# marcobellagente93/scaling

Measured on AMD Instinct MI355X. Metric: tokens/sec (whole node) Llama-2-7B-shape bf16, TP×PP×DP on 1/2/4/8 MI355X, higher is better.
Workload: dtype bf16

## Files before the change

csrc/bindings.cpp:

```cpp
#include <torch/extension.h>
#include <ATen/hip/HIPContext.h>
#include <c10/core/DeviceGuard.h>

#include <atomic>
#include <cmath>
#include <cstring>
#include <string>
#include <vector>
#include "kernels/launch.h"

void register_rehearsal(pybind11::module& m);
void register_blaslt(pybind11::module& m);

namespace {

hipStream_t cur_stream() { return at::hip::getCurrentHIPStream().stream(); }

int dt(const at::Tensor& t) {
    switch (t.scalar_type()) {
        case at::kFloat: return DT_F32;
        case at::kBFloat16: return DT_BF16;
        case at::kHalf: return DT_F16;
        default: TORCH_CHECK(false, "scaling_amd: unsupported dtype ", t.scalar_type());
    }
    return -1;
}

void check_cuda(const at::Tensor& t, const char* name) {
    TORCH_CHECK(t.is_cuda(), "scaling_amd: ", name, " must be a GPU tensor");
    TORCH_CHECK(t.is_contiguous(), "scaling_amd: ", name, " must be contiguous");
}

std::vector<at::Tensor> norm_fwd(const at::Tensor& x, const at::Tensor& w, const c10::optional<at::Tensor>& b,
                                 double eps, bool layer, const c10::optional<at::Tensor>& res) {
    check_cuda(x, "x");
    check_cuda(w, "weight");
    const int64_t H = x.size(-1);
    TORCH_CHECK(H % 8 == 0, "norm: hidden size must be a multiple of 8");
    TORCH_CHECK(w.numel() == H && w.scalar_type() == x.scalar_type(), "norm: weight shape/dtype mismatch");
    const int64_t rows = x.numel() / H;
    const at::DeviceGuard g(x.device());
    auto y = at::empty_like(x);
    auto opts = x.options().dtype(at::kFloat);
    auto rstd = at::empty({rows}, opts);
    auto mean = layer ? at::empty({rows}, opts) : at::empty({0}, opts);
    const void* bp = nullptr;
    if (layer) {
        TORCH_CHECK(b.has_value(), "layernorm needs a bias");
        check_cuda(*b, "bias");
        bp = b->data_ptr();
    }
    at::Tensor sum = at::empty({0}, x.options());
    const void* rp = nullptr;
    if (res.has_value()) {
        check_cuda(*res, "residual");
        TORCH_CHECK(res->sizes() == x.sizes() && res->scalar_type() == x.scalar_type(), "norm: residual mismatch");
        sum = at::empty_like(x);
        rp = res->data_ptr();
    }
    sa_launch::norm_fwd(dt(x), layer, x.data_ptr(), w.data_ptr(), bp, y.data_ptr(),
                        layer ? mean.data_ptr<float>() : nullptr, rstd.data_ptr<float>(), rows, (int)H, (float)eps,
// ... 311 lines not shown
    const int64_t M = x.size(0), K = W.size(1), N = epi == 2 ? W.size(0) / 2 : W.size(0);
    const at::DeviceGuard g(x.device());
    at::Tensor s = x;
    const void* ap = nullptr;
    if (add.has_value() && add->defined()) {
        TORCH_CHECK(add->sizes() == x.sizes() && add->is_contiguous() && add->scalar_type() == x.scalar_type() &&
                        (uintptr_t)add->data_ptr() % 16 == 0, "gemv_norm: add must be a contiguous, aligned [M, K]");
        s = at::empty_like(x);
        ap = add->data_ptr();
    }
    auto y = at::empty({M, N}, x.options());
    sa_launch::gemv(dt(x), (int)M, x.data_ptr(), x.stride(0), W.data_ptr(), W.stride(0), nullptr, y.data_ptr(), N, (int)N,
                    (int)K, cur_stream(), (int)epi, nullptr, 0, gamma.data_ptr(), ap, ap ? s.data_ptr() : nullptr,
                    (float)eps);
    return {s, y};
}
c10::optional<at::Tensor> gemv_norm_rope(const at::Tensor& x, const at::Tensor& gamma, double eps, const at::Tensor& W,
                                         const at::Tensor& cosb, const at::Tensor& sinb, const at::Tensor& pos,
                                         int64_t nq, int64_t nkv, int64_t rd, at::Tensor kc, at::Tensor vc,
                                         at::Tensor err) {
    TORCH_CHECK(err_word(err), "gemv_norm_rope: err must be an int32 GPU tensor");
    if (!gemv_norm_ok(x, W, gamma) || x.size(0) != 1) return c10::nullopt;
    if (!(kc.is_cuda() && kc.dim() == 3 && kc.is_contiguous() && vc.is_contiguous() && vc.sizes() == kc.sizes() &&
          kc.size(1) == nkv && kc.scalar_type() == x.scalar_type() && vc.scalar_type() == x.scalar_type()))
        return c10::nullopt;
    const int64_t hd = kc.size(2);
    if (hd % 2 || rd % 2 || rd > hd || W.size(0) != (nq + 2 * nkv) * hd) return c10::nullopt;
    if (!(pos.is_cuda() && pos.scalar_type() == at::kLong && pos.numel() == 1 && cosb.scalar_type() == at::kFloat &&
          sinb.scalar_type() == at::kFloat && cosb.is_contiguous() && sinb.is_contiguous() && cosb.size(-1) == rd / 2 &&
          sinb.sizes() == cosb.sizes()))
        return c10::nullopt;
    const at::DeviceGuard g(x.device());
    auto q = at::empty({1, nq, hd}, x.options());
    GemvRope r{cosb.data_ptr<float>(), sinb.data_ptr<float>(), pos.data_ptr<int64_t>(), q.data_ptr(), kc.data_ptr(),
               vc.data_ptr(), (int)nq, (int)nkv, (int)hd, (int)rd, std::min<int64_t>(kc.size(0), cosb.size(0)),
               err.data_ptr<int>()};
    sa_launch::gemv(dt(x), 1, x.data_ptr(), x.stride(0), W.data_ptr(), W.stride(0), nullptr, nullptr, 0,
                    (int)W.size(0), (int)W.size(1), cur_stream(), 3, nullptr, 0, gamma.data_ptr(), nullptr, nullptr,
                    (float)eps, &r);
    return q;
}

bool gemm_tn_ok(const at::Tensor& A, const at::Tensor& B, const at::Tensor& C) {
    if (!(A.is_cuda() && B.is_cuda() && C.is_cuda() && A.dim() == 2 && B.dim() == 2 && C.dim() == 2)) return false;
    if (A.scalar_type() != at::kBFloat16 || B.scalar_type() != at::kBFloat16 || C.scalar_type() != at::kBFloat16)
        return false;
    if (A.stride(1) != 1 || B.stride(1) != 1 || C.stride(1) != 1 || A.size(0) != B.size(0) || C.size(0) != A.size(1) ||
        C.size(1) != B.size(1))
        return false;
    for (const at::Tensor* t : {&A, &B}) if ((uintptr_t)t->data_ptr() % 16 != 0) return false;
    if ((uintptr_t)C.data_ptr() % 8 != 0) return false;
    return sa_launch::gemm_tn_supported(A.size(1), B.size(1), A.size(0), A.stride(0), B.stride(0), C.stride(0));
}
void gemm_tn(const at::Tensor& A, const at::Tensor& B, const at::Tensor& C, bool accumulate) {
    TORCH_CHECK(gemm_tn_ok(A, B, C), "gemm_tn: unsupported operands (bf16 2-D, M/N multiples of 16, K of 128)");
    const at::DeviceGuard g(A.device());
    static int slots = -1;
    if (slots < 0) {
        hipDeviceProp_t prop;
        slots = hipGetDeviceProperties(&prop, A.device().index()) == hipSuccess ? prop.multiProcessorCount : 0;
    }
    int full_blocks = -1, split = 1;
    const int64_t ws_floats = sa_launch::gemm_tn_plan(A.size(1), B.size(1), A.size(0), slots, full_blocks, split);
    at::Tensor ws;
    if (ws_floats > 0) ws = at::empty({ws_floats}, A.options().dtype(at::kFloat));
    sa_launch::gemm_tn(A.data_ptr(), A.stride(0), B.data_ptr(), B.stride(0), C.data_ptr(), C.stride(0), A.size(1),
                       B.size(1), A.size(0), accumulate, cur_stream(), full_blocks, split,
                       ws_floats > 0 ? ws.data_ptr<float>() : nullptr);
}

void check_qkv(const at::Tensor& t, const char* n) {
    TORCH_CHECK(t.is_cuda() && t.dim() == 3 && t.stride(2) == 1, "flash_attn: ", n, " must be [T, heads, D] with unit last stride");
    TORCH_CHECK(t.scalar_type() == at::kBFloat16 || t.scalar_type() == at::kHalf, "flash_attn: ", n, " must be bfloat16 or float16");
    TORCH_CHECK(t.stride(1) % 8 == 0 && t.stride(0) % 8 == 0, "flash_attn: ", n, " strides must be multiples of 8");
}
uint32_t drop_threshold(double p) {
    const double t = p * 4294967296.0;
    return t >= 4294967295.0 ? 0xffffffffu : (uint32_t)t;
}
std::vector<at::Tensor> fa_fwd(const at::Tensor& q, const at::Tensor& k, const at::Tensor& v, const at::Tensor& cu_q,
                               const at::Tensor& cu_k, int64_t max_q, double scale, bool causal, int64_t window,
                               double p_drop, int64_t seed, int64_t local_heads, int64_t max_k) {
    check_qkv(q, "q"); check_qkv(k, "k"); check_qkv(v, "v");
    TORCH_CHECK(k.scalar_type() == q.scalar_type() && v.scalar_type() == q.scalar_type(), "flash_attn: q/k/v dtypes differ");
    TORCH_CHECK(p_drop >= 0.0 && p_drop < 1.0, "flash_attn: dropout probability must be in [0, 1)");
    const int64_t D = q.size(2);
    TORCH_CHECK(D == 32 || D == 64 || D == 128, "flash_attn: head dim must be 32, 64 or 128");
    TORCH_CHECK(k.size(2) == D && v.size(2) == D && k.size(1) == v.size(1) && q.size(1) % k.size(1) == 0, "flash_attn: shapes");
    TORCH_CHECK(cu_q.scalar_type() == at::kInt && cu_k.scalar_type() == at::kInt && cu_q.numel() == cu_k.numel(), "flash_attn: cu_seqlens int32");
    const at::DeviceGuard g(q.device());
    const int64_t T = q.size(0), H = q.size(1);
    auto o = at::empty({T, H, D}, q.options());
    auto lse = at::empty({H, T}, q.options().dtype(at::kFloat));
    FwdArgs a{};
    a.q = (const uint16_t*)q.data_ptr(); a.k = (const uint16_t*)k.data_ptr(); a.v = (const uint16_t*)v.data_ptr();
    a.o = (uint16_t*)o.data_ptr(); a.lse = lse.data_ptr<float>();
    a.q_tok = q.stride(0); a.q_head = q.stride(1); a.k_tok = k.stride(0); a.k_head = k.stride(1);
    a.v_tok = v.stride(0); a.v_head = v.stride(1); a.o_tok = o.stride(0); a.o_head = o.stride(1); a.lse_stride = T;
    a.cu_q = cu_q.data_ptr<int>(); a.cu_k = cu_k.data_ptr<int>();
    a.nseg = (int)cu_q.numel() - 1; a.Hq = (int)H; a.Hkv = (int)k.size(1); a.causal = causal ? 1 : 0; a.window = (int)window;
    a.local_heads = local_heads < 0 ? (int)H : (int)local_heads;
    a.scale_log2 = (float)(scale * 1.4426950408889634);
    a.p_drop = (float)p_drop; a.rp_drop = (float)(1.0 / (1.0 - p_drop)); a.seed = (uint32_t)seed; a.drop_thr = drop_threshold(p_drop);
    const int64_t grp = H / k.size(1);
    if (T > 0 && a.nseg > 0 && p_drop == 0.0 && max_q * grp <= 32) {
        DecArgs d{};
        d.q = a.q; d.k = a.k; d.v = a.v;
        d.q_tok = a.q_tok; d.q_head = a.q_head; d.k_tok = a.k_tok; d.k_head = a.k_head; d.v_tok = a.v_tok; d.v_head = a.v_head;
        d.cu_q = a.cu_q; d.cu_k = a.cu_k; d.nseg = a.nseg; d.Hq = a.Hq; d.Hkv = a.Hkv; d.causal = a.causal;
        d.window = a.window; d.local_heads = a.local_heads; d.scale_log2 = a.scale_log2; d.Tq = T;
        sa_launch::fa_decode_plan(max_k > 0 ? max_k : k.size(0), a.Hkv, a.nseg, d.split_keys, d.nsplit);
        auto part_o = at::empty({(int64_t)d.nsplit, T, H, D}, q.options().dtype(at::kFloat));
        auto part_ml = at::empty({(int64_t)d.nsplit, T, H, 2}, q.options().dtype(at::kFloat));
        d.part_o = part_o.data_ptr<float>(); d.part_ml = part_ml.data_ptr<float>();
        d.o = a.o; d.o_tok = a.o_tok; d.o_head = a.o_head; d.lse = a.lse; d.lse_stride = a.lse_stride;
        sa_launch::fa_decode(d, (int)D, q.scalar_type() == at::kHalf, cur_stream());
        return {o, lse};
    }
    if (T > 0 && a.nseg > 0) sa_launch::fa_fwd(a, (int)D, (int)max_q, q.scalar_type() == at::kHalf, cur_stream());
    return {o, lse};
}
// ... 192 lines not shown
    TORCH_CHECK(logits.stride(1) == 1 || V == 1, "sample: logits need a unit last stride");
    TORCH_CHECK(B <= 1 || logits.stride(0) >= 0, "sample: negative row stride");
    TORCH_CHECK(step.is_cuda() && step.scalar_type() == at::kLong && step.numel() == 1 &&
                step.device() == logits.device(), "sample: step must be one int64 on the logits' device");
    TORCH_CHECK(temperature > 0.0 && std::isfinite(temperature), "sample: temperature must be positive");
    TORCH_CHECK(!std::isnan(top_p), "sample: top_p is NaN");
    const int code = dt(logits);
    const at::DeviceGuard g(logits.device());
    auto tokens = at::empty({B}, logits.options().dtype(at::kLong));
    at::Tensor info;
    if (want_info) info = at::empty({B, 2}, logits.options().dtype(at::kInt));
    if (B > 0)
        sa_launch::sample(code, logits.data_ptr(), B > 1 ? logits.stride(0) : 0, B, (int)V, tokens.data_ptr<int64_t>(),
                          want_info ? info.data_ptr<int>() : nullptr, step.data_ptr<int64_t>(), (uint32_t)seed,
                          (int)std::max<int64_t>(0, std::min<int64_t>(top_k, V)), (float)std::max(top_p, 0.0),
                          (float)temperature, cur_stream());
    if (want_info) return {tokens, info};
    return {tokens};
}
}

PYBIND11_MODULE(TORCH_EXTENSION_NAME, m) {
    m.def("sample_logits", &sample_logits, "one draw per row of logits [B, V] after top-k / top-p / temperature "
          "(graph-safe: the step is read on the device)", py::arg("logits"), py::arg("step"), py::arg("seed"),
          py::arg("temperature"), py::arg("top_k"), py::arg("top_p"), py::arg("want_info") = false);
    m.def("sample_max_resident_vocab", []() { return sa_launch::sample_max_resident(); },
          "the largest vocabulary whose row the sampling kernel stages in LDS");
    m.doc() = "scaling_amd CDNA4 (gfx950) HIP kernels";
    register_rehearsal(m);
    register_blaslt(m);
    m.def("norm_fwd", &norm_fwd, "RMSNorm/LayerNorm forward (optional fused residual add)", py::arg("x"), py::arg("w"), py::arg("b"), py::arg("eps"), py::arg("layer"), py::arg("res") = py::none());
    m.def("norm_bwd", &norm_bwd, "RMSNorm/LayerNorm backward (optional fused residual-gradient add)", py::arg("dy"), py::arg("x"), py::arg("w"), py::arg("mean"), py::arg("rstd"), py::arg("layer"), py::arg("dadd") = py::none());
    m.def("swiglu_fwd", &swiglu_fwd, "SwiGLU forward");
    m.def("swiglu_bwd", &swiglu_bwd, "SwiGLU backward");
    m.def("ar_alloc", &ar_alloc, "one-shot all-reduce: allocate + IPC-export a registered buffer");
    m.def("ar_open", &ar_open, "one-shot all-reduce: map a peer's registered buffer");
    m.def("ar_close", &ar_close, "unmap a peer buffer");
    m.def("ar_free", &ar_free, "free an own registered buffer");
    m.def("ar_allreduce", &ar_allreduce, "one-shot all-reduce of x over the registered buffers (in place)",
          py::arg("x"), py::arg("bases"), py::arg("rank"), py::arg("slot_off"), py::arg("flag_off"), py::arg("epoch"),
          py::arg("signal"), py::arg("err"), py::arg("max_spins") = int64_t(1) << 26);
    m.def("transpose_ok", &transpose_ok, "whether transpose2d supports this tensor");
    m.def("transpose2d", &transpose2d, "x^T (contiguous) for 2-byte 2-D matrices");
    m.def("gemv_ok", &gemv_ok, "whether gemv supports these operands");
    m.def("gemv", &gemv, "y = x W^T (+ b) for at most 4 rows of x (decode-time linear layers)", py::arg("x"), py::arg("W"), py::arg("bias") = py::none());
    m.def("gemv_residual", &gemv_residual, "y = x W^T + res for at most 4 rows (decode MLP-out + residual)");
    m.def("gemv_swiglu", &gemv_swiglu, "y = silu(x Wg^T) * (x Wu^T) for W = [Wg; Wu], at most 4 rows (decode)");
    m.def("gemv_norm_ok", &gemv_norm_ok, "whether gemv_norm supports these operands");
    m.def("gemv_norm_rope", &gemv_norm_rope, "graph decode: rms_norm + q/k/v GEMV + interleaved RoPE + K/V cache append "
          "in one launch; returns q or None");
    m.def("gemv_norm", &gemv_norm, "(s, gemv(rms_norm(s), W)) with s = x (+ add); epi 0 plain, 2 SwiGLU (decode)",
          py::arg("x"), py::arg("add"), py::arg("gamma"), py::arg("eps"), py::arg("W"), py::arg("epi") = 0);
    m.def("gemm_tn_ok", &gemm_tn_ok, "whether gemm_tn supports these operands");
    m.def("gemm_tn", &gemm_tn, "C (+)= A^T B for k-major bf16 operands (weight-gradient GEMM)");
    m.def("rope", &rope, "rotary embedding (fwd / inverse), optional strided / in-place output", py::arg("x"), py::arg("cos"), py::arg("sin"), py::arg("pos"), py::arg("rot_dim"), py::arg("seq_len"), py::arg("interleaved"), py::arg("inverse"), py::arg("out") = py::none());
    m.def("rope_kv_append", &rope_kv_append, "graph decode: RoPE q, RoPE k into the K cache row, v into the V cache row");
    m.def("xent_stats", &xent_stats, "cross-entropy row statistics");
    m.def("xent_bwd", &xent_bwd, "cross-entropy backward");
    m.def("embed_fwd", &embed_fwd, "vocab-parallel embedding forward");
    m.def("embed_bwd", &embed_bwd, "deterministic embedding backward", py::call_guard<py::gil_scoped_release>());
    m.def("adamw_", &adamw_, "fused AdamW on flat fp32 buffers");
    m.def("sumsq_", &sumsq_, "sum of squares + non-finite count");
    m.def("cast_scale_", &cast_scale_, "y = cast(x * scale)");
    m.def("masked_softmax_fwd", &masked_softmax_fwd, "softmax(masked_fill(x * scale, mask, fill)) over the last dim", py::arg("x"), py::arg("mask"), py::arg("scale"), py::arg("fill"), py::arg("round_scaled"));
    m.def("masked_softmax_bwd", &masked_softmax_bwd, "masked softmax backward", py::arg("dy"), py::arg("y"), py::arg("mask"), py::arg("scale"));
    m.def("act_fwd", &act_fwd, "activation forward (0 gelu, 1 silu, 2 gelu-tanh)");
    m.def("act_bwd", &act_bwd, "activation backward");
    m.def("spin_us", &spin_us, "debug: busy-wait kernel of ~us microseconds on the current stream");
    m.def("gate_flags_alloc", &gate_flags_alloc, "stream gates: n flag words (coherent pinned host memory)");
    m.def("gate_flag_write", &gate_flag_write, "stream gates: host store of a flag word (after a full fence)");
    m.def("gate_flag_read", &gate_flag_read, "stream gates: host load of a flag word");
    m.def("gate_stream_wait", &gate_stream_wait, "stream gates: the current stream waits until flag[idx] >= value");
    m.def("xgmi_emulate", &xgmi_emulate, "per-rank proxy: emulated collective (HBM traffic on nwg CUs, held to us)",
          py::arg("src"), py::arg("scratch"), py::arg("bytes"), py::arg("us"), py::arg("nwg") = 16);
    m.def("dropout_add", &dropout_add, "residual + dropout(x) with a hashed keep mask", py::arg("x"), py::arg("res"), py::arg("p"), py::arg("seed"));
    m.def("fa_fwd", &fa_fwd, "flash attention forward (bf16/fp16, optional attention dropout)", py::arg("q"), py::arg("k"), py::arg("v"), py::arg("cu_q"), py::arg("cu_k"), py::arg("max_q"), py::arg("scale"), py::arg("causal"), py::arg("window"), py::arg("p_drop") = 0.0, py::arg("seed") = 0, py::arg("local_heads") = -1, py::arg("max_k") = -1);
    m.def("fa_bwd", &fa_bwd, "flash attention backward (optional strided dq/dk/dv outputs)", py::arg("dout"), py::arg("q"), py::arg("k"), py::arg("v"), py::arg("o"), py::arg("lse"), py::arg("cu_q"), py::arg("cu_k"), py::arg("max_q"), py::arg("max_k"), py::arg("scale"), py::arg("causal"), py::arg("window"), py::arg("dq_out") = py::none(), py::arg("dk_out") = py::none(), py::arg("dv_out") = py::none(), py::arg("p_drop") = 0.0, py::arg("seed") = 0, py::arg("local_heads") = -1, py::arg("rope_cos") = py::none(), py::arg("rope_sin") = py::none(), py::arg("rope_pos") = py::none(), py::arg("rope_dim") = 0, py::arg("rope_seq") = 1, py::arg("rope_interleaved") = false);
}
```

csrc/kernels/gemm.hip:

```cpp
#include <algorithm>

#include "common.h"
#include "flash_attn.h"
#include "launch.h"

using namespace sa;

namespace sa_gemm {

using fa::bf16x8;
using fa::lds_s16x4;
using fa::lds_void;

__host__ __device__ __forceinline__ int group_m(int tm, int tn) {
#ifdef SA_WGRAD_GROUPM
    (void)tm;
    (void)tn;
    return SA_WGRAD_GROUPM;
#else
    return tm >= 2 * tn ? 4 : 8;
#endif
}
constexpr int BK = 32;
constexpr int kImg = BK * 256 * 2;
constexpr int kSlot = 2 * kImg;
constexpr int kSlots = 4;
constexpr int NW = 4;
constexpr int NP = kImg / 1024 / NW;

template <int N>
__device__ __forceinline__ void wait_vm() {
    asm volatile("s_waitcnt vmcnt(%0)" ::"n"(N) : "memory");
}
__device__ __forceinline__ void hard_barrier() {
    __builtin_amdgcn_sched_barrier(0);
    asm volatile("s_barrier" ::: "memory");
    __builtin_amdgcn_sched_barrier(0);
}
__device__ __forceinline__ void mfma16_acc(f32x4& c, const bf16x8& a, const bf16x8& b) {
    asm volatile("v_mfma_f32_16x16x32_bf16 %0, %1, %2, %0" : "+a"(c) : "v"(a), "v"(b));
}
__device__ __forceinline__ int sw16(int r) { return ((r & 3) << 2) ^ (((r >> 2) & 1) << 1); }
__device__ __forceinline__ int koff16(int r, int c) { return r * 512 + 16 * ((c >> 3) ^ sw16(r)) + ((c & 7) << 1); }

#ifndef SA_WGRAD_ROUND
#define SA_WGRAD_ROUND 1
#endif
__device__ __forceinline__ int round_remap(int b, int nwg) {
    if constexpr (SA_WGRAD_ROUND) {
        constexpr int R = 256;
        const int full = nwg / R * R;
        if (b >= full) return full + xcd_remap(b - full, nwg - full);
        return b / R * R + xcd_remap(b % R, R);
    }
    return xcd_remap(b, nwg);
}

template <bool BETA>
__global__ __launch_bounds__(256, 1) void gemm_tn_ring_kernel(const u16* __restrict__ A, int lda, uint32_t a_bytes,
                                                              const u16* __restrict__ B, int ldb, uint32_t b_bytes,
                                                              u16* __restrict__ C, int ldc, int M, int N, int K,
                                                              int full_blocks, int tail_split, float* __restrict__ ws) {
    extern __shared__ __attribute__((aligned(16))) char smem[];
    const int lane = threadIdx.x & 63;
    const int wave = __builtin_amdgcn_readfirstlane(threadIdx.x >> 6);
    const int wm = wave >> 1, wn = wave & 1;

    const int tm = (M + 255) / 256, tn = (N + 255) / 256;
    int v, k_lo = 0, nk = K / 64, unit = -1;
    if ((int)blockIdx.x < full_blocks) {
        v = round_remap(blockIdx.x, full_blocks);
    } else {
        unit = (int)blockIdx.x - full_blocks;
        v = full_blocks + unit / tail_split;
        nk /= tail_split;
        k_lo = (unit % tail_split) * nk;
    }
    const int ns = 2 * nk, s_lo = 2 * k_lo;
    const int gM = group_m(tm, tn);
    const int group = gM * tn;
    const int first_m = (v / group) * gM;
    const int gm = min(tm - first_m, gM);
    const int within = v % group;
    const int m0 = (first_m + within % gm) * 256, n0 = (within / gm) * 256;

    int voff_a, voff_b, step_a, step_b;
    {
        const int row = 2 * wave + (lane >> 5);
        const int slot = (lane & 31) ^ sw16(row);
        voff_a = (row * lda + slot * 8) * 2;
        voff_b = (row * ldb + slot * 8) * 2;
        step_a = __builtin_amdgcn_readfirstlane(4 * NW * lda);
        step_b = __builtin_amdgcn_readfirstlane(4 * NW * ldb);
    }
    auto soff_a = [&](int u) { return __builtin_amdgcn_readfirstlane(((s_lo + min(u, ns - 1)) * BK * lda + m0) * 2); };
    auto soff_b = [&](int u) { return __builtin_amdgcn_readfirstlane(((s_lo + min(u, ns - 1)) * BK * ldb + n0) * 2); };
    typedef int i32x4 __attribute__((ext_vector_type(4)));
    const i32x4 rsa = {(int)__builtin_amdgcn_readfirstlane((uint32_t)reinterpret_cast<uint64_t>(A)),
                       (int)(__builtin_amdgcn_readfirstlane((uint32_t)(reinterpret_cast<uint64_t>(A) >> 32)) & 0xffff),
                       (int)__builtin_amdgcn_readfirstlane(a_bytes), fa::kBufFlags};
    const i32x4 rsb = {(int)__builtin_amdgcn_readfirstlane((uint32_t)reinterpret_cast<uint64_t>(B)),
                       (int)(__builtin_amdgcn_readfirstlane((uint32_t)(reinterpret_cast<uint64_t>(B) >> 32)) & 0xffff),
                       (int)__builtin_amdgcn_readfirstlane(b_bytes), fa::kBufFlags};
    const uint32_t lds0 = __builtin_amdgcn_readfirstlane((uint32_t)reinterpret_cast<uintptr_t>((lds_void*)smem));
#define SA_RING_PIECE(P, SLOT, SA, SB)                                                                           \
    {                                                                                                            \
        const int i_ = (P) >> 1;                                                                                 \
        const uint32_t l_ = lds0 + (SLOT) * kSlot + (((P) & 1) ? kImg : 0) + (wave + NW * i_) * 1024;            \
        if ((P) & 1)                                                                                             \
            asm volatile("s_mov_b32 m0, %0\n\ts_nop 0\n\tbuffer_load_dwordx4 %1, %2, %3 offen lds" ::"s"(l_),    \
                         "v"(voff_b), "s"(rsb), "s"((SB) + i_ * step_b)                                       \
                         : "m0");                                                                                \
        else                                                                                                     \
            asm volatile("s_mov_b32 m0, %0\n\ts_nop 0\n\tbuffer_load_dwordx4 %1, %2, %3 offen lds" ::"s"(l_),    \
                         "v"(voff_a), "s"(rsa), "s"((SA) + i_ * step_a)                                       \
                         : "m0");                                                                                \
    }
#define SA_RING_MFMA_PIECE(C_, A_, B_, P, SLOT, SA, SB)                                                          \
    {                                                                                                            \
        const int i_ = (P) >> 1;                                                                                 \
        const uint32_t l_ = lds0 + (SLOT) * kSlot + (((P) & 1) ? kImg : 0) + (wave + NW * i_) * 1024;            \
        if ((P) & 1)                                                                                             \
            asm volatile("s_mov_b32 m0, %3\n\tv_mfma_f32_16x16x32_bf16 %0, %1, %2, %0\n\t"                     \
                         "buffer_load_dwordx4 %4, %5, %6 offen lds"                                              \
                         : "+a"(C_) : "v"(A_), "v"(B_), "s"(l_), "v"(voff_b), "s"(rsb), "s"((SB) + i_ * step_b)  \
                         : "m0");                                                                                \
        else                                                                                                     \
            asm volatile("s_mov_b32 m0, %3\n\tv_mfma_f32_16x16x32_bf16 %0, %1, %2, %0\n\t"                     \
                         "buffer_load_dwordx4 %4, %5, %6 offen lds"                                              \
                         : "+a"(C_) : "v"(A_), "v"(B_), "s"(l_), "v"(voff_a), "s"(rsa), "s"((SA) + i_ * step_a)  \
                         : "m0");                                                                                \
    }

    f32x4 acc[8][8];
#pragma unroll
    for (int i = 0; i < 8; ++i)
#pragma unroll
        for (int j = 0; j < 8; ++j) acc[i][j] = f32x4{0.f, 0.f, 0.f, 0.f};

    int oa[2][8], ob[2][8];
    {
        const int g = lane >> 4, i16 = lane & 15;
        const int row = 4 * g + (i16 >> 2), cl = 4 * (i16 & 3);
#pragma unroll
        for (int h = 0; h < 2; ++h)
#pragma unroll
            for (int i = 0; i < 8; ++i) {
                oa[h][i] = h * 2 * kSlot + koff16(row, 128 * wm + 16 * i + cl);
                ob[h][i] = h * 2 * kSlot + kImg + koff16(row, 128 * wn + 16 * i + cl);
            }
    }
    auto frag = [&](int off, int slot) -> bf16x8 {
        const char* p = smem + off + (slot & 1) * kSlot;
        const s16x4 x = __builtin_amdgcn_ds_read_tr16_b64_v4i16((lds_s16x4*)p);
        const s16x4 y = __builtin_amdgcn_ds_read_tr16_b64_v4i16((lds_s16x4*)(p + 16 * 512));
        return __builtin_bit_cast(bf16x8, __builtin_shufflevector(x, y, 0, 1, 2, 3, 4, 5, 6, 7));
    };
    bf16x8 fa0[8], fb0[8], fa1[8], fb1[8];
#define SA_RING_READ(SLOT, FA, FB, F)                                         \
    {                                                                         \
        if ((F) < 8) FB[(F)] = frag(ob[(SLOT) >> 1][(F)], (SLOT));            \
        else FA[(F) - 8] = frag(oa[(SLOT) >> 1][(F) - 8], (SLOT));            \
    }
#define SA_RING_STEP(SLOT, T, FA, FB, NA, NB)                                                                   \
    {                                                                                                           \
        const int sa_ = soff_a((T) + 4), sb_ = soff_b((T) + 4);                                                 \
        _Pragma("unroll") for (int i = 0; i < 8; ++i)                                                           \
            _Pragma("unroll") for (int j = 0; j < 8; ++j) {                                                     \
                const int m_ = i * 8 + j;                                                                       \
                if ((m_ & 7) == 3) SA_RING_MFMA_PIECE(acc[i][j], FB[j], FA[i], m_ >> 3, SLOT, sa_, sb_)         \
                else mfma16_acc(acc[i][j], FB[j], FA[i]);                                                       \
                if ((m_ & 3) == 1) SA_RING_READ(((SLOT) + 1) & 3, NA, NB, m_ >> 2)                              \
            }                                                                                                   \
        asm volatile("s_waitcnt lgkmcnt(0)" ::: "memory");                                                      \
        wait_vm<4 * NP>();                                                                                      \
        hard_barrier();                                                                                         \
    }

    asm volatile("s_nop 4" ::: "memory");
#pragma unroll
    for (int u = 0; u < 4; ++u) {
        const int sa_ = soff_a(u), sb_ = soff_b(u);
#pragma unroll
        for (int p = 0; p < 8; ++p) SA_RING_PIECE(p, u, sa_, sb_)
    }
    wait_vm<4 * NP>();
    hard_barrier();
#pragma unroll
    for (int f = 0; f < 16; ++f) SA_RING_READ(0, fa0, fb0, f)
    asm volatile("s_waitcnt lgkmcnt(0)" ::: "memory");
    hard_barrier();
    for (int t = 0; t + 3 < ns; t += 4) {
        SA_RING_STEP(0, t, fa0, fb0, fa1, fb1)
        SA_RING_STEP(1, t + 1, fa1, fb1, fa0, fb0)
        SA_RING_STEP(2, t + 2, fa0, fb0, fa1, fb1)
        SA_RING_STEP(3, t + 3, fa1, fb1, fa0, fb0)
    }
#undef SA_RING_STEP
#undef SA_RING_READ
#undef SA_RING_PIECE
#undef SA_RING_MFMA_PIECE
    wait_vm<0>();
    asm volatile("s_nop 7\n\ts_nop 7\n\ts_nop 7" ::: "memory");
#pragma unroll
    for (int i = 0; i < 8; ++i)
#pragma unroll
        for (int j = 0; j < 8; ++j) asm volatile("" : "+a"(acc[i][j]));

    const int r = lane & 15, q4 = 4 * (lane >> 4);
    if (unit >= 0) {
        float* wp = ws + (int64_t)unit * 65536;
#pragma unroll
        for (int i = 0; i < 8; ++i) {
            float* rp = wp + (128 * wm + 16 * i + r) * 256 + 128 * wn + q4;
#pragma unroll
            for (int j = 0; j < 8; ++j) *reinterpret_cast<f32x4*>(rp + 16 * j) = acc[i][j];
        }
        return;
    }
    const bool edge = m0 + 256 > M || n0 + 256 > N;
#pragma unroll
    for (int i = 0; i < 8; ++i) {
        if (edge && m0 + 128 * wm + 16 * i >= M) continue;
        u16* crow_p = C + (int64_t)(m0 + 128 * wm + 16 * i + r) * ldc + n0 + 128 * wn + q4;
        u16x4 old[8];
        if (BETA) {
#pragma unroll
            for (int j = 0; j < 8; ++j)
                if (!edge || n0 + 128 * wn + 16 * j < N) old[j] = *reinterpret_cast<const u16x4*>(crow_p + 16 * j);
        }
#pragma unroll
        for (int j = 0; j < 8; ++j) {
            if (edge && n0 + 128 * wn + 16 * j >= N) continue;
            u16x4 o;
#pragma unroll
            for (int e = 0; e < 4; ++e) {
                float x = acc[i][j][e];
                if (BETA) x += bf2f(old[j][e]);
                o[e] = f2bf(x);
            }
            *reinterpret_cast<u16x4*>(crow_p + 16 * j) = o;
        }
    }
}
template __global__ void gemm_tn_ring_kernel<true>(const u16* __restrict__, int, uint32_t, const u16* __restrict__, int,
                                                   uint32_t, u16* __restrict__, int, int, int, int, int, int,
                                                   float* __restrict__);
template __global__ void gemm_tn_ring_kernel<false>(const u16* __restrict__, int, uint32_t, const u16* __restrict__, int,
                                                    uint32_t, u16* __restrict__, int, int, int, int, int, int,
                                                    float* __restrict__);

__global__ __launch_bounds__(256) void gemm_tn_combine_kernel(const float* __restrict__ ws, u16* __restrict__ C, int ldc,
                                                              int M, int N, int full_blocks, int split, int beta) {
    const int tm = (M + 255) / 256, tn = (N + 255) / 256;
    const int v = full_blocks + (int)blockIdx.x;
    const int gM = group_m(tm, tn);
    const int group = gM * tn;
    const int first_m = (v / group) * gM;
    const int gm = min(tm - first_m, gM);
    const int within = v % group;
    const int m0 = (first_m + within % gm) * 256, n0 = (within / gm) * 256;
    const int row = 4 * (int)blockIdx.y + (threadIdx.x >> 6), col = (threadIdx.x & 63) * 4;
    if (m0 + row >= M || n0 + col >= N) return;
    f32x4 acc = {0.f, 0.f, 0.f, 0.f};
    const float* wp = ws + (int64_t)blockIdx.x * split * 65536 + row * 256 + col;
    for (int p = 0; p < split; ++p) {
        const f32x4 x = *reinterpret_cast<const f32x4*>(wp + (int64_t)p * 65536);
        acc += x;
    }
    u16* cp = C + (int64_t)(m0 + row) * ldc + n0 + col;
    u16x4 o;
    const u16x4 old = beta ? *reinterpret_cast<const u16x4*>(cp) : u16x4{0, 0, 0, 0};
#pragma unroll
    for (int e = 0; e < 4; ++e) o[e] = f2bf(acc[e] + (beta ? bf2f(old[e]) : 0.f));
    *reinterpret_cast<u16x4*>(cp) = o;
}

}
using namespace sa_gemm;

namespace sa_launch {
bool gemm_tn_supported(int64_t M, int64_t N, int64_t K, int64_t lda, int64_t ldb, int64_t ldc) {
    return M % 16 == 0 && N % 16 == 0 && K % 128 == 0 && M > 0 && N > 0 && K > 0 && lda % 8 == 0 &&
           ldb % 8 == 0 && ldc % 4 == 0 && K * lda * 2 < (int64_t(1) << 31) && K * ldb * 2 < (int64_t(1) << 31) &&
           ldc < (1 << 30);
}
int64_t gemm_tn_plan(int64_t M, int64_t N, int64_t K, int slots, int& full_blocks, int& split) {
    const int nwg = (int)(((M + 255) / 256) * ((N + 255) / 256));
    full_blocks = nwg;
    split = 1;
    if (slots <= 0) return 0;
    const int r = nwg % slots, nk = (int)(K / 64);
    if (r == 0 || nk % 2 != 0) return 0;
    int s = 1;
    double best = 1.0;
    for (int c = 2; c <= 4; ++c) {
        if (nk % c != 0 || nk / c < 4 || (nk / c) % 2 != 0) continue;
        const double cost = (double)((r * c + slots - 1) / slots) / c;
        if (cost < best - 1e-9) { best = cost; s = c; }
    }
    if (s <= 1 || best > 0.8) return 0;
    split = s;
    full_blocks = nwg - r;
    return (int64_t)r * s * 65536;
}
void gemm_tn(const void* A, int64_t lda, const void* B, int64_t ldb, void* C, int64_t ldc, int64_t M, int64_t N,
             int64_t K, bool beta, hipStream_t st, int full_blocks, int split, float* ws) {
    const int nwg = (int)(((M + 255) / 256) * ((N + 255) / 256));
    if (full_blocks < 0 || split <= 1) { full_blocks = nwg; split = 1; }
    const int grid = full_blocks + (nwg - full_blocks) * split;
    const uint32_t ab = (uint32_t)(K * lda * 2), bb = (uint32_t)(K * ldb * 2);
    if (beta)
        hipLaunchKernelGGL((gemm_tn_ring_kernel<true>), dim3(grid), dim3(256), kSlots * kSlot, st, (const u16*)A,
                           (int)lda, ab, (const u16*)B, (int)ldb, bb, (u16*)C, (int)ldc, (int)M, (int)N, (int)K,
                           full_blocks, split, ws);
    else
        hipLaunchKernelGGL((gemm_tn_ring_kernel<false>), dim3(grid), dim3(256), kSlots * kSlot, st, (const u16*)A,
                           (int)lda, ab, (const u16*)B, (int)ldb, bb, (u16*)C, (int)ldc, (int)M, (int)N, (int)K,
                           full_blocks, split, ws);
    if (split > 1)
        hipLaunchKernelGGL(gemm_tn_combine_kernel, dim3(nwg - full_blocks, 64), dim3(256), 0, st, (const float*)ws,
                           (u16*)C, (int)ldc, (int)M, (int)N, full_blocks, split, beta ? 1 : 0);
}
}
```

csrc/kernels/launch.h:

```cpp
#pragma once
#include <hip/hip_runtime.h>
#include <stdint.h>

enum SaDType { DT_F32 = 0, DT_BF16 = 1, DT_F16 = 2 };

namespace sa_launch {
void norm_fwd(int dtype, bool layer, const void* x, const void* w, const void* b, void* y, float* mean, float* rstd,
              int64_t rows, int H, float eps, hipStream_t st, const void* res = nullptr, void* sum_out = nullptr);
int norm_bwd_waves(int64_t rows, int H);
int64_t norm_bwd_scratch(int64_t rows, int H, bool layer);
void norm_bwd(int dtype, bool layer, const void* dy, const void* x, const void* w, const float* mean,
              const float* rstd, void* dx, void* dw, void* db, float* part, int64_t rows, int H, hipStream_t st,
              const void* dadd = nullptr);
}

namespace sa_launch {
void swiglu_fwd(int dtype, const void* a, const void* b, int64_t lda, void* out, int64_t rows, int F, hipStream_t st);
void swiglu_bwd(int dtype, const void* dy, const void* a, const void* b, int64_t lda, void* da, void* db, int64_t ldd,
                int64_t rows, int F, hipStream_t st);
void rope(int dtype, bool interleaved, const void* x, int64_t x_tok, int64_t x_head, void* out, int64_t o_tok,
          int64_t o_head, const float* cosb, const float* sinb, const int64_t* pos, int64_t T_, int nh, int hd, int rd,
          int seq_len, float sign, hipStream_t st);
bool rope_kv_append(int dtype, bool interleaved, const void* x, void* q_out, void* kc, void* vc, const int64_t* pos,
                    const float* cosb, const float* sinb, int nq, int nkv, int hd, int rd, int64_t lim, int* err,
                    hipStream_t st);
}

namespace sa_launch {
void xent_stats(int dtype, const void* logits, const int64_t* tgt, int64_t rows, int V, int64_t v0, float* m, float* s,
                float* t, int64_t* amax, hipStream_t st);
void xent_bwd(int dtype, const void* logits, const int64_t* tgt, const float* lse, const float* gscale, void* dlogits,
              int64_t rows, int V, int64_t v0, hipStream_t st);
void embed_fwd(int dtype, const int64_t* ids, const void* W, void* out, int64_t ntok, int H, int64_t v0, int64_t Vp,
               hipStream_t st);
void embed_bwd(int dtype, const void* dy, const int64_t* order, const int64_t* sid, int64_t ntok, void* dW, int H,
               int64_t v0, int64_t Vp, hipStream_t st);
void adamw(int gdtype, int pdtype, float* p, const void* g, float* m, float* v, void* pout, int64_t n, float lr,
           float b1, float b2, float eps, float wd, float bc1, float bc2_sqrt, float gscale, hipStream_t st);
int sumsq_blocks(int64_t n);
void sumsq(int dtype, const void* x, int64_t n, float scale, float* part_sq, float* part_bad, float* out_sq,
           float* out_bad, int accumulate, hipStream_t st);
void cast_scale(int sdt, int ddt, const void* x, void* y, int64_t n, float scale, hipStream_t st);
bool transpose_supported(int64_t R, int64_t C, int64_t ld_in);
void transpose_u16(const void* in, int64_t ld_in, void* out, int64_t R, int64_t C, hipStream_t st);
}

namespace sa_launch {
bool gemm_tn_supported(int64_t M, int64_t N, int64_t K, int64_t lda, int64_t ldb, int64_t ldc);
int64_t gemm_tn_plan(int64_t M, int64_t N, int64_t K, int slots, int& full_blocks, int& split);
void gemm_tn(const void* A, int64_t lda, const void* B, int64_t ldb, void* C, int64_t ldc, int64_t M, int64_t N,
             int64_t K, bool beta, hipStream_t st, int full_blocks = -1, int split = 1, float* ws = nullptr);
}

struct FwdArgs {
    const uint16_t* q; const uint16_t* k; const uint16_t* v; uint16_t* o; float* lse;
    int64_t q_tok, q_head, k_tok, k_head, v_tok, v_head, o_tok, o_head, lse_stride;
    const int* cu_q; const int* cu_k;
    int nseg, Hq, Hkv, causal, window;
    int local_heads;
    float scale_log2;
    float p_drop, rp_drop;
    uint32_t seed, drop_thr;
};
namespace sa_launch {
void fa_fwd(const FwdArgs& a, int D, int max_q, bool f16, hipStream_t st);
}

struct DecArgs {
    const uint16_t* q; const uint16_t* k; const uint16_t* v;
    int64_t q_tok, q_head, k_tok, k_head, v_tok, v_head;
    const int* cu_q; const int* cu_k;
    int nseg, Hq, Hkv, causal, window, local_heads;
    float scale_log2;
    int split_keys, nsplit;
    int64_t Tq;
    float* part_o;
    float* part_ml;
    uint16_t* o; int64_t o_tok, o_head;
    float* lse; int64_t lse_stride;
};
namespace sa_launch {
void fa_decode_plan(int64_t max_k, int Hkv, int nseg, int& split_keys, int& nsplit);
void fa_decode(const DecArgs& a, int D, bool f16, hipStream_t st);
}

struct BwdArgs {
    const uint16_t* q; const uint16_t* k; const uint16_t* v; const uint16_t* dO;
    const float* lse; float* delta; float* lse2;
    uint16_t* dq; uint16_t* dk; uint16_t* dv;
    int64_t q_tok, q_head, k_tok, k_head, v_tok, v_head, do_tok, do_head;
    int64_t dq_tok, dq_head, dk_tok, dk_head, dv_tok, dv_head, lse_stride;
    const int* cu_q; const int* cu_k;
    int nseg, Hq, Hkv, causal, window;
    int local_heads;
    float scale, scale_log2;
    float p_drop, rp_drop;
    uint32_t seed, drop_thr;
    int hsplit, Tk;
    float* dk_part;
    float* dv_part;
    const float* rcos; const float* rsin; const int64_t* rpos;
    int rrd, rseq, ril;
};
namespace sa_launch {
// ... 43 lines not shown
```

Baseline: 33110.

## Replace split-K tail plan with stream-K style chunk balancing for gemm_tn

The weight-gradient GEMM's last partial wave used to be split into 2-4 equal K pieces per tile. It is now handled by distributing every K chunk of the tail tiles evenly over all workgroup slots, so a workgroup may cover parts of several tiles. Each segment writes an fp32 partial to its own workspace slot, and the combine kernel sums a tile's range of slots. A cost model decides whether the tail split pays off, and the slot count can be overridden. The intent is to remove tail-wave underutilisation, at the cost of extra workspace traffic and a combine launch.

Result: no change. 33170 (median of 6 runs) (+0.2%).

```diff
diff --git a/csrc/bindings.cpp b/csrc/bindings.cpp
--- a/csrc/bindings.cpp
+++ b/csrc/bindings.cpp
@@ -7,6 +7,7 @@
 #include <cstring>
 #include <string>
 #include <vector>
+#include "kernels/gemm_tn_plan.h"
 #include "kernels/launch.h"
 
 void register_rehearsal(pybind11::module& m);
@@ -424,21 +425,22 @@
     if ((uintptr_t)C.data_ptr() % 8 != 0) return false;
     return sa_launch::gemm_tn_supported(A.size(1), B.size(1), A.size(0), A.stride(0), B.stride(0), C.stride(0));
 }
-void gemm_tn(const at::Tensor& A, const at::Tensor& B, const at::Tensor& C, bool accumulate) {
+void gemm_tn(const at::Tensor& A, const at::Tensor& B, const at::Tensor& C, bool accumulate, int64_t slots) {
     TORCH_CHECK(gemm_tn_ok(A, B, C), "gemm_tn: unsupported operands (bf16 2-D, M/N multiples of 16, K of 128)");
+    TORCH_CHECK(slots >= -1 && slots <= 4096, "gemm_tn: slots must be -1 (the device's CU count) or 0..4096");
     const at::DeviceGuard g(A.device());
-    static int slots = -1;
-    if (slots < 0) {
+    static int cus = -1;
+    if (cus < 0) {
         hipDeviceProp_t prop;
-        slots = hipGetDeviceProperties(&prop, A.device().index()) == hipSuccess ? prop.multiProcessorCount : 0;
-    }
-    int full_blocks = -1, split = 1;
-    const int64_t ws_floats = sa_launch::gemm_tn_plan(A.size(1), B.size(1), A.size(0), slots, full_blocks, split);
+        cus = hipGetDeviceProperties(&prop, A.device().index()) == hipSuccess ? prop.multiProcessorCount : 0;
+    }
+    const int s = slots < 0 ? cus : (int)slots;
+    const int64_t ws_floats =
+        sa_gemm_plan::workspace_floats(sa_gemm_plan::make_plan(A.size(1), B.size(1), A.size(0), s));
     at::Tensor ws;
     if (ws_floats > 0) ws = at::empty({ws_floats}, A.options().dtype(at::kFloat));
     sa_launch::gemm_tn(A.data_ptr(), A.stride(0), B.data_ptr(), B.stride(0), C.data_ptr(), C.stride(0), A.size(1),
-                       B.size(1), A.size(0), accumulate, cur_stream(), full_blocks, split,
-                       ws_floats > 0 ? ws.data_ptr<float>() : nullptr);
+                       B.size(1), A.size(0), accumulate, cur_stream(), s, ws_floats > 0 ? ws.data_ptr<float>() : nullptr);
 }
 
 void check_qkv(const at::Tensor& t, const char* n) {
@@ -737,7 +739,9 @@
     m.def("gemv_norm", &gemv_norm, "(s, gemv(rms_norm(s), W)) with s = x (+ add); epi 0 plain, 2 SwiGLU (decode)",
           py::arg("x"), py::arg("add"), py::arg("gamma"), py::arg("eps"), py::arg("W"), py::arg("epi") = 0);
     m.def("gemm_tn_ok", &gemm_tn_ok, "whether gemm_tn supports these operands");
-    m.def("gemm_tn", &gemm_tn, "C (+)= A^T B for k-major bf16 operands (weight-gradient GEMM)");
+    m.def("gemm_tn", &gemm_tn, "C (+)= A^T B for k-major bf16 operands (weight-gradient GEMM); slots: workgroup slots "
+          "the tail of the last round is planned for (-1: the device's CU count)", py::arg("A"), py::arg("B"),
+          py::arg("C"), py::arg("accumulate"), py::arg("slots") = -1);
     m.def("rope", &rope, "rotary embedding (fwd / inverse), optional strided / in-place output", py::arg("x"), py::arg("cos"), py::arg("sin"), py::arg("pos"), py::arg("rot_dim"), py::arg("seq_len"), py::arg("interleaved"), py::arg("inverse"), py::arg("out") = py::none());
     m.def("rope_kv_append", &rope_kv_append, "graph decode: RoPE q, RoPE k into the K cache row, v into the V cache row");
     m.def("xent_stats", &xent_stats, "cross-entropy row statistics");
diff --git a/csrc/kernels/gemm.hip b/csrc/kernels/gemm.hip
--- a/csrc/kernels/gemm.hip
+++ b/csrc/kernels/gemm.hip
@@ -2,6 +2,7 @@
 
 #include "common.h"
 #include "flash_attn.h"
+#include "gemm_tn_plan.h"
 #include "launch.h"
 
 using namespace sa;
@@ -60,29 +61,35 @@
 __global__ __launch_bounds__(256, 1) void gemm_tn_ring_kernel(const u16* __restrict__ A, int lda, uint32_t a_bytes,
                                                               const u16* __restrict__ B, int ldb, uint32_t b_bytes,
                                                               u16* __restrict__ C, int ldc, int M, int N, int K,
-                                                              int full_blocks, int tail_split, float* __restrict__ ws) {
+                                                              sa_gemm_plan::Plan plan, float* __restrict__ ws) {
     extern __shared__ __attribute__((aligned(16))) char smem[];
     const int lane = threadIdx.x & 63;
     const int wave = __builtin_amdgcn_readfirstlane(threadIdx.x >> 6);
     const int wm = wave >> 1, wn = wave & 1;
 
     const int tm = (M + 255) / 256, tn = (N + 255) / 256;
-    int v, k_lo = 0, nk = K / 64, unit = -1;
-    if ((int)blockIdx.x < full_blocks) {
-        v = round_remap(blockIdx.x, full_blocks);
-    } else {
-        unit = (int)blockIdx.x - full_blocks;
-        v = full_blocks + unit / tail_split;
-        nk /= tail_split;
-        k_lo = (unit % tail_split) * nk;
-    }
-    const int ns = 2 * nk, s_lo = 2 * k_lo;
+    const int unit = (int)blockIdx.x - plan.full_blocks;
+    const int nseg = unit >= 0 ? sa_gemm_plan::segment_count(plan, unit) : 1;
     const int gM = group_m(tm, tn);
     const int group = gM * tn;
-    const int first_m = (v / group) * gM;
-    const int gm = min(tm - first_m, gM);
-    const int within = v % group;
-    const int m0 = (first_m + within % gm) * 256, n0 = (within / gm) * 256;
+    int m0 = 0, n0 = 0, s_lo = 0, ns = K / BK, pslot = 0;
+    auto set_segment = [&](int sg) {
+        int v;
+        if (unit < 0) {
+            v = round_remap(blockIdx.x, plan.full_blocks);
+        } else {
+            const sa_gemm_plan::Segment s = sa_gemm_plan::segment(plan, unit, sg);
+            v = plan.full_blocks + sa_gemm_plan::tail_tile_order(plan, s.tile);
+            s_lo = __builtin_amdgcn_readfirstlane(4 * s.first_chunk);
+            ns = __builtin_amdgcn_readfirstlane(4 * s.chunks);
+            pslot = __builtin_amdgcn_readfirstlane(s.slot);
+        }
+        const int first_m = (v / group) * gM;
+        const int gm = min(tm - first_m, gM);
+        const int within = v % group;
+        m0 = (first_m + within % gm) * 256;
+        n0 = (within / gm) * 256;
+    };
 
     int voff_a, voff_b, step_a, step_b;
     {
@@ -133,10 +140,6 @@
     }
 
     f32x4 acc[8][8];
-#pragma unroll
-    for (int i = 0; i < 8; ++i)
-#pragma unroll
-        for (int j = 0; j < 8; ++j) acc[i][j] = f32x4{0.f, 0.f, 0.f, 0.f};
 
     int oa[2][8], ob[2][8];
     {
@@ -177,47 +180,55 @@
         hard_barrier();                                                                                         \
     }
 
-    asm volatile("s_nop 4" ::: "memory");
-#pragma unroll
-    for (int u = 0; u < 4; ++u) {
-        const int sa_ = soff_a(u), sb_ = soff_b(u);
-#pragma unroll
-        for (int p = 0; p < 8; ++p) SA_RING_PIECE(p, u, sa_, sb_)
-    }
-    wait_vm<4 * NP>();
-    hard_barrier();
-#pragma unroll
-    for (int f = 0; f < 16; ++f) SA_RING_READ(0, fa0, fb0, f)
-    asm volatile("s_waitcnt lgkmcnt(0)" ::: "memory");
-    hard_barrier();
-    for (int t = 0; t + 3 < ns; t += 4) {
-        SA_RING_STEP(0, t, fa0, fb0, fa1, fb1)
-        SA_RING_STEP(1, t + 1, fa1, fb1, fa0, fb0)
-        SA_RING_STEP(2, t + 2, fa0, fb0, fa1, fb1)
-        SA_RING_STEP(3, t + 3, fa1, fb1, fa0, fb0)
+    const int r = lane & 15, q4 = 4 * (lane >> 4);
+    for (int sg = 0;; ++sg) {
+        set_segment(sg);
+#pragma unroll
+        for (int i = 0; i < 8; ++i)
+#pragma unroll
+            for (int j = 0; j < 8; ++j) acc[i][j] = f32x4{0.f, 0.f, 0.f, 0.f};
+        asm volatile("s_nop 4" ::: "memory");
+#pragma unroll
+        for (int u = 0; u < 4; ++u) {
+            const int sa_ = soff_a(u), sb_ = soff_b(u);
+#pragma unroll
+            for (int p = 0; p < 8; ++p) SA_RING_PIECE(p, u, sa_, sb_)
+        }
+        wait_vm<4 * NP>();
+        hard_barrier();
+#pragma unroll
+        for (int f = 0; f < 16; ++f) SA_RING_READ(0, fa0, fb0, f)
+        asm volatile("s_waitcnt lgkmcnt(0)" ::: "memory");
+        hard_barrier();
+        for (int t = 0; t + 3 < ns; t += 4) {
+            SA_RING_STEP(0, t, fa0, fb0, fa1, fb1)
+            SA_RING_STEP(1, t + 1, fa1, fb1, fa0, fb0)
+            SA_RING_STEP(2, t + 2, fa0, fb0, fa1, fb1)
+            SA_RING_STEP(3, t + 3, fa1, fb1, fa0, fb0)
+        }
+        wait_vm<0>();
+        asm volatile("s_nop 7\n\ts_nop 7\n\ts_nop 7" ::: "memory");
+#pragma unroll
+        for (int i = 0; i < 8; ++i)
+#pragma unroll
+            for (int j = 0; j < 8; ++j) asm volatile("" : "+a"(acc[i][j]));
+        if (unit < 0) break;
+        float* wp = ws + (int64_t)pslot * sa_gemm_plan::kTileFloats;
+#pragma unroll
+        for (int i = 0; i < 8; ++i) {
+            float* rp = wp + (128 * wm + 16 * i + r) * 256 + 128 * wn + q4;
+#pragma unroll
+            for (int j = 0; j < 8; ++j) *reinterpret_cast<f32x4*>(rp + 16 * j) = acc[i][j];
+        }
+        if (sg + 1 >= nseg) return;
+        asm volatile("s_waitcnt lgkmcnt(0)" ::: "memory");
+        hard_barrier();
     }
 #undef SA_RING_STEP
 #undef SA_RING_READ
 #undef SA_RING_PIECE
 #undef SA_RING_MFMA_PIECE
-    wait_vm<0>();
-    asm volatile("s_nop 7\n\ts_nop 7\n\ts_nop 7" ::: "memory");
-#pragma unroll
-    for (int i = 0; i < 8; ++i)
-#pragma unroll
-        for (int j = 0; j < 8; ++j) asm volatile("" : "+a"(acc[i][j]));
-
-    const int r = lane & 15, q4 = 4 * (lane >> 4);
-    if (unit >= 0) {
-        float* wp = ws + (int64_t)unit * 65536;
-#pragma unroll
-        for (int i = 0; i < 8; ++i) {
-            float* rp = wp + (128 * wm + 16 * i + r) * 256 + 128 * wn + q4;
-#pragma unroll
-            for (int j = 0; j < 8; ++j) *reinterpret_cast<f32x4*>(rp + 16 * j) = acc[i][j];
-        }
-        return;
-    }
+
     const bool edge = m0 + 256 > M || n0 + 256 > N;
 #pragma unroll
     for (int i = 0; i < 8; ++i) {
@@ -244,16 +255,16 @@
     }
 }
 template __global__ void gemm_tn_ring_kernel<true>(const u16* __restrict__, int, uint32_t, const u16* __restrict__, int,
-                                                   uint32_t, u16* __restrict__, int, int, int, int, int, int,
+                                                   uint32_t, u16* __restrict__, int, int, int, int, sa_gemm_plan::Plan,
                                                    float* __restrict__);
 template __global__ void gemm_tn_ring_kernel<false>(const u16* __restrict__, int, uint32_t, const u16* __restrict__, int,
-                                                    uint32_t, u16* __restrict__, int, int, int, int, int, int,
+                                                    uint32_t, u16* __restrict__, int, int, int, int, sa_gemm_plan::Plan,
                                                     float* __restrict__);
 
 __global__ __launch_bounds__(256) void gemm_tn_combine_kernel(const float* __restrict__ ws, u16* __restrict__ C, int ldc,
-                                                              int M, int N, int full_blocks, int split, int beta) {
+                                                              int M, int N, sa_gemm_plan::Plan plan, int beta) {
     const int tm = (M + 255) / 256, tn = (N + 255) / 256;
-    const int v = full_blocks + (int)blockIdx.x;
+    const int v = plan.full_blocks + sa_gemm_plan::tail_tile_order(plan, (int)blockIdx.x);
     const int gM = group_m(tm, tn);
     const int group = gM * tn;
     const int first_m = (v / group) * gM;
@@ -263,9 +274,11 @@
     const int row = 4 * (int)blockIdx.y + (threadIdx.x >> 6), col = (threadIdx.x & 63) * 4;
     if (m0 + row >= M || n0 + col >= N) return;
     f32x4 acc = {0.f, 0.f, 0.f, 0.f};
-    const float* wp = ws + (int64_t)blockIdx.x * split * 65536 + row * 256 + col;
-    for (int p = 0; p < split; ++p) {
-        const f32x4 x = *reinterpret_cast<const f32x4*>(wp + (int64_t)p * 65536);
+    int first, last;
+    sa_gemm_plan::tile_slots(plan, (int)blockIdx.x, first, last);
+    const float* wp = ws + row * 256 + col;
+    for (int p = first; p <= last; ++p) {
+        const f32x4 x = *reinterpret_cast<const f32x4*>(wp + (int64_t)p * sa_gemm_plan::kTileFloats);
         acc += x;
     }
     u16* cp = C + (int64_t)(m0 + row) * ldc + n0 + col;
@@ -285,41 +298,21 @@
            ldb % 8 == 0 && ldc % 4 == 0 && K * lda * 2 < (int64_t(1) << 31) && K * ldb * 2 < (int64_t(1) << 31) &&
            ldc < (1 << 30);
 }
-int64_t gemm_tn_plan(int64_t M, int64_t N, int64_t K, int slots, int& full_blocks, int& split) {
-    const int nwg = (int)(((M + 255) / 256) * ((N + 255) / 256));
-    full_blocks = nwg;
-    split = 1;
-    if (slots <= 0) return 0;
-    const int r = nwg % slots, nk = (int)(K / 64);
-    if (r == 0 || nk % 2 != 0) return 0;
-    int s = 1;
-    double best = 1.0;
-    for (int c = 2; c <= 4; ++c) {
-        if (nk % c != 0 || nk / c < 4 || (nk / c) % 2 != 0) continue;
-        const double cost = (double)((r * c + slots - 1) / slots) / c;
-        if (cost < best - 1e-9) { best = cost; s = c; }
-    }
-    if (s <= 1 || best > 0.8) return 0;
-    split = s;
-    full_blocks = nwg - r;
-    return (int64_t)r * s * 65536;
-}
 void gemm_tn(const void* A, int64_t lda, const void* B, int64_t ldb, void* C, int64_t ldc, int64_t M, int64_t N,
-             int64_t K, bool beta, hipStream_t st, int full_blocks, int split, float* ws) {
-    const int nwg = (int)(((M + 255) / 256) * ((N + 255) / 256));
-    if (full_blocks < 0 || split <= 1) { full_blocks = nwg; split = 1; }
-    const int grid = full_blocks + (nwg - full_blocks) * split;
+             int64_t K, bool beta, hipStream_t st, int slots, float* ws) {
+    const sa_gemm_plan::Plan plan = sa_gemm_plan::make_plan(M, N, K, ws != nullptr ? slots : 0);
+    const int grid = plan.full_blocks + plan.tail_wgs;
     const uint32_t ab = (uint32_t)(K * lda * 2), bb = (uint32_t)(K * ldb * 2);
     if (beta)
         hipLaunchKernelGGL((gemm_tn_ring_kernel<true>), dim3(grid), dim3(256), kSlots * kSlot, st, (const u16*)A,
-                           (int)lda, ab, (const u16*)B, (int)ldb, bb, (u16*)C, (int)ldc, (int)M, (int)N, (int)K,
-                           full_blocks, split, ws);
+                           (int)lda, ab, (const u16*)B, (int)ldb, bb, (u16*)C, (int)ldc, (int)M, (int)N, (int)K, plan,
+                           ws);
     else
         hipLaunchKernelGGL((gemm_tn_ring_kernel<false>), dim3(grid), dim3(256), kSlots * kSlot, st, (const u16*)A,
-                           (int)lda, ab, (const u16*)B, (int)ldb, bb, (u16*)C, (int)ldc, (int)M, (int)N, (int)K,
-                           full_blocks, split, ws);
-    if (split > 1)
-        hipLaunchKernelGGL(gemm_tn_combine_kernel, dim3(nwg - full_blocks, 64), dim3(256), 0, st, (const float*)ws,
-                           (u16*)C, (int)ldc, (int)M, (int)N, full_blocks, split, beta ? 1 : 0);
-}
-}
+                           (int)lda, ab, (const u16*)B, (int)ldb, bb, (u16*)C, (int)ldc, (int)M, (int)N, (int)K, plan,
+                           ws);
+    if (plan.tail_wgs > 0)
+        hipLaunchKernelGGL(gemm_tn_combine_kernel, dim3(plan.tail_tiles, 64), dim3(256), 0, st, (const float*)ws,
+                           (u16*)C, (int)ldc, (int)M, (int)N, plan, beta ? 1 : 0);
+}
+}
diff --git a/csrc/kernels/gemm_tn_plan.h b/csrc/kernels/gemm_tn_plan.h
--- /dev/null
+++ b/csrc/kernels/gemm_tn_plan.h
@@ -0,0 +1,82 @@
+#pragma once
+#include <cstdint>
+
+namespace sa_gemm_plan {
+
+constexpr int kTile = 256;
+constexpr int kChunk = 128;
+constexpr int kTileFloats = kTile * kTile;
+constexpr int64_t kNsPerK = 22, kNsPerPartial = 105, kNsCombineLaunch = 5000;
+
+struct Plan {
+    int full_blocks;
+    int tail_tiles;
+    int chunks;
+    int tail_wgs;
+    int tail_group;
+};
+struct Segment {
+    int tile;
+    int first_chunk;
+    int chunks;
+    int slot;
+};
+
+constexpr int tile_count(int64_t M, int64_t N) { return (int)(((M + kTile - 1) / kTile) * ((N + kTile - 1) / kTile)); }
+
+constexpr Plan make_plan(int64_t M, int64_t N, int64_t K, int slots) {
+    const int tiles = tile_count(M, N);
+    Plan p = {tiles, 0, (int)(K / kChunk), 0, 0};
+    if (slots <= 0 || K % kChunk != 0) return p;
+    const int r = tiles % slots;
+    if (r == 0 || (int64_t)r * p.chunks < slots || (int64_t)r * p.chunks >= (int64_t(1) << 30)) return p;
+    const int64_t saved = (int64_t)(slots - r) * K * kNsPerK;
+    const int64_t cost = (int64_t)slots * ((int64_t)(slots + r - 1) * kNsPerPartial + kNsCombineLaunch);
+    if (saved <= cost) return p;
+    p.full_blocks = tiles - r;
+    p.tail_tiles = r;
+    p.tail_wgs = slots;
+    int a = r, b = slots;
+    while (b != 0) {
+        const int c = a % b;
+        a = b;
+        b = c;
+    }
+    p.tail_group = a;
+    return p;
+}
+
+constexpr int tail_tile_order(const Plan& p, int t) {
+    const int per = p.tail_tiles / p.tail_group;
+    return (t % per) * p.tail_group + t / per;
+}
+
+constexpr int64_t workspace_floats(const Plan& p) {
+    return p.tail_wgs > 0 ? (int64_t)(p.tail_wgs + p.tail_tiles - 1) * kTileFloats : 0;
+}
+
+constexpr int share_begin(const Plan& p, int w) {
+    const int total = p.tail_tiles * p.chunks, q = total / p.tail_wgs, rem = total % p.tail_wgs;
+    return w * q + (w < rem ? w : rem);
+}
+constexpr int chunk_owner(const Plan& p, int g) {
+    const int total = p.tail_tiles * p.chunks, q = total / p.tail_wgs, rem = total % p.tail_wgs;
+    const int big = rem * (q + 1);
+    return g < big ? g / (q + 1) : rem + (g - big) / q;
+}
+constexpr int segment_count(const Plan& p, int w) {
+    return (share_begin(p, w + 1) - 1) / p.chunks - share_begin(p, w) / p.chunks + 1;
+}
+constexpr Segment segment(const Plan& p, int w, int s) {
+    const int g0 = share_begin(p, w), g1 = share_begin(p, w + 1);
+    const int tile = g0 / p.chunks + s;
+    const int lo = g0 > tile * p.chunks ? g0 : tile * p.chunks;
+    const int hi = g1 < (tile + 1) * p.chunks ? g1 : (tile + 1) * p.chunks;
+    return Segment{tile, lo - tile * p.chunks, hi - lo, w + tile};
+}
+constexpr void tile_slots(const Plan& p, int t, int& first, int& last) {
+    first = chunk_owner(p, t * p.chunks) + t;
+    last = chunk_owner(p, (t + 1) * p.chunks - 1) + t;
+}
+
+}
diff --git a/csrc/kernels/launch.h b/csrc/kernels/launch.h
--- a/csrc/kernels/launch.h
+++ b/csrc/kernels/launch.h
@@ -47,9 +47,8 @@
 
 namespace sa_launch {
 bool gemm_tn_supported(int64_t M, int64_t N, int64_t K, int64_t lda, int64_t ldb, int64_t ldc);
-int64_t gemm_tn_plan(int64_t M, int64_t N, int64_t K, int slots, int& full_blocks, int& split);
 void gemm_tn(const void* A, int64_t lda, const void* B, int64_t ldb, void* C, int64_t ldc, int64_t M, int64_t N,
-             int64_t K, bool beta, hipStream_t st, int full_blocks = -1, int split = 1, float* ws = nullptr);
+             int64_t K, bool beta, hipStream_t st, int slots = 0, float* ws = nullptr);
 }
 
 struct FwdArgs {
```
